# mynameisfiber/baton

Measured on NVIDIA H100. Metric: federated local samples/sec (whole box), ResNet-18 FedAvg, synthetic non-IID 32x32 shards, higher is better.
Workload: dtype bf16

## Files before the change

### baton_b200/csrc/bindings.cpp

```cpp
#include <ATen/cuda/CUDAContext.h>
#include <c10/cuda/CUDAGuard.h>
#include <torch/extension.h>

#include <optional>
#include <vector>

#include "launch.h"

namespace {

inline cudaStream_t cur_stream() { return at::cuda::getCurrentCUDAStream().stream(); }
inline void check(int rc, const char* what) {
  TORCH_CHECK(rc == 0, "baton_b200::", what, " failed with code ", rc,
              rc > 0 ? std::string(" (") + cudaGetErrorString(static_cast<cudaError_t>(rc)) + ")" : std::string());
}
inline const void* cptr(const at::Tensor& t) { return t.data_ptr(); }
inline void* ptr(at::Tensor& t) { return t.data_ptr(); }
template <class T>
inline T* opt_ptr(const std::optional<at::Tensor>& t) {
  return (t.has_value() && t->defined()) ? reinterpret_cast<T*>(t->data_ptr()) : nullptr;
}
#define CHECK_CUDA(x) TORCH_CHECK((x).is_cuda(), #x " must be a CUDA tensor")

inline const float* prox_anchor(const std::optional<at::Tensor>& anchor, int64_t numel, const at::Tensor& hyper) {
// ... 248 lines not shown
  return true;
}
bool conv_smallmap(const at::Tensor& src, const at::Tensor& w, at::Tensor out, int64_t stride, bool dgrad, int64_t mc,
                   int64_t bn, const std::optional<at::Tensor>& col_stats) {
  CHECK_CUDA(src); CHECK_CUDA(w); CHECK_CUDA(out);
  TORCH_CHECK(src.scalar_type() == at::kBFloat16 && w.scalar_type() == at::kBFloat16 && out.scalar_type() == at::kBFloat16 &&
              src.dim() == 4 && src.is_contiguous() && w.is_contiguous() && out.is_contiguous());
  TORCH_CHECK(stride == 1 || stride == 2, "conv_smallmap: stride 1 or 2");
  const int64_t c = src.size(3);
  const int64_t rows = src.size(0) * ((src.size(1) - 1) / stride + 1) * ((src.size(2) - 1) / stride + 1);
  TORCH_CHECK(rows > 0 && out.numel() % rows == 0, "conv_smallmap: out must hold [N*Ho*Wo, Nout] elements");
  const int64_t nout = out.numel() / rows;
  TORCH_CHECK(w.numel() == (dgrad ? c * 9 * nout : nout * 9 * c), "conv_smallmap: w must be [Cout, 9*Cin]");
  TORCH_CHECK(dgrad ? !col_stats.has_value()
                    : (!col_stats.has_value() || (col_stats->scalar_type() == at::kFloat && col_stats->numel() >= 2 * nout)),
              "conv_smallmap: col_stats is a [2 Cout] fp32 buffer of the forward");
  const c10::cuda::CUDAGuard guard(src.device());
  const int rc = b200_conv_smallmap(cptr(src), cptr(w), ptr(out), static_cast<int>(src.size(0)),
                                    static_cast<int>(src.size(1)), static_cast<int>(src.size(2)), static_cast<int>(c),
                                    static_cast<int>(nout), static_cast<int>(stride), dgrad ? 1 : 0, static_cast<int>(mc),
                                    static_cast<int>(bn), opt_ptr<float>(col_stats), cur_stream());
  if (rc == -2) return false;
  check(rc, "conv_smallmap");
  return true;
}
bool conv_igemm_dgrad_s2(const at::Tensor& dy, const at::Tensor& w, at::Tensor dx, int64_t kh, int64_t kw,
                         const std::vector<int64_t>& ntaps, const std::vector<int64_t>& taps, int64_t force_bn) {
  CHECK_CUDA(dy); CHECK_CUDA(w); CHECK_CUDA(dx);
  TORCH_CHECK(dy.scalar_type() == at::kBFloat16 && w.scalar_type() == at::kBFloat16 && dx.scalar_type() == at::kBFloat16 &&
              dy.dim() == 4 && dx.dim() == 4 && dy.is_contiguous() && w.is_contiguous() && dx.is_contiguous());
  TORCH_CHECK(ntaps.size() == 4 && taps.size() == 16, "conv_igemm_dgrad_s2: 4 classes x 4 taps");
  int nt[4], tw[16];
  for (int i = 0; i < 4; ++i) nt[i] = static_cast<int>(ntaps[i]);
  for (int i = 0; i < 16; ++i) tw[i] = static_cast<int>(taps[i]);
  const c10::cuda::CUDAGuard guard(dy.device());
  const int rc = b200_conv_igemm_dgrad_s2(cptr(dy), cptr(w), ptr(dx), static_cast<int>(dx.size(0)),
                                          static_cast<int>(dx.size(1)), static_cast<int>(dx.size(2)),
                                          static_cast<int>(dx.size(3)), static_cast<int>(dy.size(3)), static_cast<int>(kh),
                                          static_cast<int>(kw), static_cast<int>(dy.size(1)), static_cast<int>(dy.size(2)),
                                          nt, tw, static_cast<int>(force_bn), cur_stream());
  if (rc == -2) return false;
  check(rc, "conv_igemm_dgrad_s2");
  return true;
}
bool conv_igemm_wgrad(const at::Tensor& dy, const at::Tensor& x, at::Tensor dw, int64_t cout, int64_t kh, int64_t kw,
                      int64_t stride, int64_t pad, int64_t ho, int64_t wo, int64_t split_k, int64_t force_bn,
// ... 1201 lines not shown

PYBIND11_MODULE(TORCH_EXTENSION_NAME, m) {
  m.doc() = "baton_b200 sm_90a kernels";
  m.attr("MAX_RANKS") = B200_MAX_RANKS;
  m.def("gemm", &gemm);
  m.def("gemm_lora", &gemm_lora);
  m.def("lora_down", &lora_down);
  m.def("lora_grad", &lora_grad);
  m.attr("LORA_MAX_R") = B200_LORA_MAX_R;
  m.attr("LORA_SPLIT_ROWS") = B200_LORA_SPLIT_ROWS;
  m.def("trace_set", &trace_set);
  m.def("attention_fwd", &attention_fwd);
  m.def("attention_bwd", &attention_bwd);
  m.def("bn_bwd_cluster", &bn_bwd_cluster);
  m.def("gn_fwd", &gn_fwd);
  m.def("gn_bwd", &gn_bwd);
  m.def("im2col_tma_probe", &im2col_tma_probe);
  m.def("conv_igemm_fwd", &conv_igemm_fwd);
  m.def("conv_igemm_wgrad", &conv_igemm_wgrad);
  m.def("conv_igemm_dgrad", &conv_igemm_dgrad);
  m.def("conv_igemm_dgrad_s2", &conv_igemm_dgrad_s2);
  m.def("conv_halo", &conv_halo);
  m.def("conv_smallmap", &conv_smallmap);
  m.def("gemm_batched", &gemm_batched);
  m.def("gemm_fp8", &gemm_fp8);
  m.def("quant_mx_rows", &quant_mx_rows);
  m.def("quant_mx_cols", &quant_mx_cols);
  m.def("fused_sgd", &fused_sgd);
  m.def("fused_sgd_segments", &fused_sgd_segments);
  m.def("grad_norm_clip", &grad_norm_clip);
  m.attr("GRAD_NORM_WORK_WORDS") = B200_GRAD_NORM_WORK_WORDS;
  m.def("weighted_sum", &weighted_sum);
  m.def("fold_client", &fold_client);
  m.def("scaffold_corr", &scaffold_corr);
  m.def("scaffold_dc", &scaffold_dc);
  m.def("cast", &cast);
  m.def("gather_rows", &gather_rows);
  m.def("gather_augment", &gather_augment);
  m.def("gather_mix", &gather_mix);
  m.def("colsum", &colsum);
  m.def("add_bf16", &add_bf16);
  m.def("relu_bwd", &relu_bwd);
  m.def("gelu", &gelu);
  m.def("gelu_bwd", &gelu_bwd);
  m.def("pad_rows", &pad_rows);
  m.def("embedding_bwd", &embedding_bwd);
// ... 51 lines not shown
```

### baton_b200/csrc/conv_halo.cu

```cuda
#define B200_TU_TAG 12
#include "ptx.cuh"
#include "epilogue.cuh"
#include "launch.h"
#include "pdl.cuh"

namespace b200 {

constexpr int HALO_BM = 64;
constexpr int HALO_BN = 64;
constexpr int HALO_TAPS = 9;
constexpr int HALO_THREADS = 256;
constexpr int HALO_CONSUMERS = 128;
constexpr int HALO_MAX_SMEM = 227 * 1024;
constexpr int HALO_ZERO_BYTES = 128;

struct HaloParams {
  int M, N;
  int Ho, Wo;
  __nv_bfloat16* D;
  float* col_stats;
  int ncol;
  int mc;
  int halo_bytes;
  int bh, bw;
};

__host__ __device__ constexpr int halo_barriers(int k_tiles) { return (1 + k_tiles + 15) / 16 * 16; }

__host__ __device__ constexpr int halo_slot_bytes(int bn) { return bn * 64 * 2; }

__host__ __device__ constexpr int halo_fixed_bytes(int k_tiles, int bn = HALO_BN, bool img = false) {
  return k_tiles * halo_slot_bytes(bn) + halo_barriers(k_tiles) * 8 + 4 * bn * 4 + (img ? HALO_ZERO_BYTES : 0) + 1024;
}

template <bool DGRAD, int CB, int STRIDE, int BN = HALO_BN, bool IMG = false>
__global__ void __launch_bounds__(HALO_THREADS, 1)
conv_halo_kernel(const __grid_constant__ CUtensorMap tmX, const __grid_constant__ CUtensorMap tmW, const HaloParams p) {
  static_assert(BN == 32 || BN == 64, "conv_halo_kernel: 32 or 64 columns");
  constexpr int KT = HALO_TAPS * CB;
  constexpr int SLOT = halo_slot_bytes(BN);
  constexpr int PITCH = BN + 4;
  constexpr int ORIGIN = IMG ? 0 : -1;
  extern __shared__ __align__(1024) uint8_t smem_raw[];
  uint8_t* smem = reinterpret_cast<uint8_t*>((reinterpret_cast<uintptr_t>(smem_raw) + 1023) & ~uintptr_t(1023));
  uint8_t* halo = smem;
  uint8_t* bslot = smem + CB * p.halo_bytes;
  uint64_t* bar = reinterpret_cast<uint64_t*>(bslot + KT * SLOT);
  float* cstat = reinterpret_cast<float*>(bar + halo_barriers(KT));
  uint8_t* zline = reinterpret_cast<uint8_t*>(cstat + 4 * BN);

  griddep_launch_dependents();
  const int warp = threadIdx.x >> 5;
  const int m0 = blockIdx.y * HALO_BM;
  const int n0 = blockIdx.x * BN;
  const int hw = p.Ho * p.Wo;
  const int hp = p.bh, wp = p.bw;

  if (warp == 0 && elect_one()) {
    tma_prefetch_desc(&tmX);
    tma_prefetch_desc(&tmW);
    for (int i = 0; i < 1 + KT; ++i) mbar_init(&bar[i], 1);
    fence_barrier_init();
  }
  __syncthreads();
  if (p.mc > 1) cluster_sync_all();
  griddep_wait();

  if (warp == 0) {
    if (elect_one()) {
      const int imgs = HALO_BM / hw;
      mbar_expect_tx(&bar[0], CB * imgs * hp * wp * 128);
#pragma unroll
      for (int cb = 0; cb < CB; ++cb)
        tma_load_4d(halo + cb * p.halo_bytes, &tmX, &bar[0], 64 * cb, ORIGIN, ORIGIN, m0 / hw);
      constexpr int SROWS = DGRAD ? 64 : BN;
      constexpr int RB = SLOT / SROWS;
      const int rows = max(SROWS / p.mc, 8);
      const int rank = p.mc > 1 ? static_cast<int>(cluster_ctarank()) : 0;
      const uint16_t mask = static_cast<uint16_t>((1u << p.mc) - 1);
#pragma unroll 1
      for (int kt = 0; kt < KT; ++kt) {
        const int tap = kt / CB, cb = kt - tap * CB;
        mbar_expect_tx(&bar[1 + kt], SLOT);
        if (rank * rows >= SROWS) continue;
        uint8_t* dst = bslot + kt * SLOT + rank * rows * RB;
        const int c0 = DGRAD ? (HALO_TAPS - 1 - tap) * p.ncol + n0 : kt * 64;
        const int c1 = DGRAD ? cb * 64 + rank * rows : n0 + rank * rows;
        if (p.mc > 1)
          tma_load_2d_mc(dst, &tmW, &bar[1 + kt], c0, c1, mask);
        else
          tma_load_2d(dst, &tmW, &bar[1 + kt], c0, c1);
      }
    }
  } else if (warp >= 4) {
    const int ew = warp - 4;
    const int lane = static_cast<int>(lane_id());
    const int m = 16 * ew + (lane & 15);
    const int img = m / hw, rem = m - img * hw;
    const int oi = rem / p.Wo, oj = rem - oi * p.Wo;
    const int y0 = STRIDE * oi - 1 - ORIGIN, x0 = STRIDE * oj - 1 - ORIGIN;
    const int hrow0 = (img * hp + y0) * wp + x0;
    const uint32_t halo_a = smem_u32(halo);
    const int half = lane >> 4;
    auto load_a = [&](uint32_t (&a)[4][4], int kt) {
      const int tap = kt / CB, cb = kt - tap * CB;
      const int r = tap / 3, s = tap - 3 * r;
      const int hrow = hrow0 + r * wp + s;
      uint32_t row_addr = halo_a + static_cast<uint32_t>(cb * p.halo_bytes + hrow * 128);
      if constexpr (IMG) {
        const int y = y0 + r, x = x0 + s;
        if (y < 0 || y >= hp || x < 0 || x >= wp) row_addr = smem_u32(zline);
      }
#pragma unroll
      for (int kk = 0; kk < 4; ++kk) ldmatrix_x4(a[kk], row_addr + ((((2 * kk + half) ^ hrow) & 7) << 4));
    };

    float acc[BN / 2];
#pragma unroll
    for (int j = 0; j < BN / 2; ++j) acc[j] = 0.f;
    uint32_t a[2][4][4];
    if constexpr (IMG) {
      if (threadIdx.x < 128 + HALO_ZERO_BYTES / 16) reinterpret_cast<uint4*>(zline)[threadIdx.x - 128] = make_uint4(0, 0, 0, 0);
      named_bar_sync(1, HALO_CONSUMERS);
    }
    mbar_wait(&bar[0], 0);
    if (threadIdx.x == 128) TRACE_POINT();
    load_a(a[0], 0);
#pragma unroll
    for (int kt = 0; kt < KT; ++kt) {
      mbar_wait(&bar[1 + kt], 0);
      if (threadIdx.x == 128 && (kt == 0 || kt == KT - 1)) TRACE_POINT();
      const uint32_t sb = smem_u32(bslot + kt * SLOT);
      wgmma_fence();
#pragma unroll
      for (int kk = 0; kk < 4; ++kk) {
        uint64_t bd;
        if constexpr (!DGRAD)
          bd = gmma_desc_sw128(sb + kk * 32, 16, 1024);
        else if constexpr (BN == 64)
          bd = gmma_desc_sw128(sb + kk * 2048, 8192, 1024);
        else
          bd = gmma_desc_sw64(sb + kk * 1024, 4096, 512);
        if constexpr (BN == 64)
          wgmma_bf16_n64_rs<DGRAD ? 1 : 0>(acc, a[kt & 1][kk], bd, 1u);
        else
          wgmma_bf16_n32_rs<DGRAD ? 1 : 0>(acc, a[kt & 1][kk], bd, 1u);
      }
      wgmma_commit();
      if (kt + 1 < KT) {
        wgmma_wait<1>();
        load_a(a[(kt + 1) & 1], kt + 1);
      }
    }
    wgmma_wait<0>();
    wgmma_fence_operands(acc);
    if (threadIdx.x == 128) TRACE_POINT();

    named_bar_sync(1, HALO_CONSUMERS);
    float* part = reinterpret_cast<float*>(smem);
    wg_store_acc<BN>(acc, part, PITCH, 0);
    named_bar_sync(1, HALO_CONSUMERS);
    const int q = ew & 1;
    const int c = (ew >> 1) * 32;
    const int lrow = q * 32 + lane;
    const int row = m0 + lrow;
    const int col0 = n0 + c;
    float* sstat = cstat + q * 2 * BN;
    const bool want_stats = p.col_stats != nullptr;
    if (c >= BN) {
    } else if (col0 >= p.N) {
      if (want_stats) { sstat[c + lane] = 0.f; sstat[BN + c + lane] = 0.f; }
    } else {
      uint32_t r[32];
      acc_ld_row32(part + lrow * PITCH + c, r);
      float v[32];
#pragma unroll
      for (int j = 0; j < 32; ++j) v[j] = __uint_as_float(r[j]);
      if (want_stats) stage_col_stats(sstat, BN, c, v);
      if (row < p.M) {
        __nv_bfloat16* d = p.D + static_cast<size_t>(row) * p.N + col0;
        if (col0 + 32 <= p.N && (p.N % 8) == 0) {
#pragma unroll
          for (int j = 0; j < 32; j += 8) {
            uint4 o;
            o.x = pack_bf16x2(v[j], v[j + 1]);
            o.y = pack_bf16x2(v[j + 2], v[j + 3]);
            o.z = pack_bf16x2(v[j + 4], v[j + 5]);
            o.w = pack_bf16x2(v[j + 6], v[j + 7]);
            *reinterpret_cast<uint4*>(d + j) = o;
          }
        } else {
          _Pragma("unroll") for (int j = 0; j < 32; ++j) if (col0 + j < p.N) d[j] = __float2bfloat16_rn(v[j]);
        }
      }
    }
    if (want_stats) {
      named_bar_sync(1, HALO_CONSUMERS);
      for (int i = threadIdx.x - 128; i < 2 * BN; i += HALO_CONSUMERS) {
        const int col = i < BN ? i : i - BN;
        if (n0 + col < p.N)
          atomicAdd(p.col_stats + (i < BN ? 0 : p.N) + n0 + col,
                    cstat[i] + cstat[2 * BN + i]);
      }
    }
  }
}

template <auto KERNEL>
static int launch_halo(const CUtensorMap& tx, const CUtensorMap& tw, const HaloParams& p, dim3 grid, int smem,
                       cudaStream_t stream) {
  static bool configured = false;
  if (!configured) {
    cudaError_t e = cudaFuncSetAttribute(KERNEL, cudaFuncAttributeMaxDynamicSharedMemorySize,
                                         HALO_MAX_SMEM);
    if (e != cudaSuccess) return static_cast<int>(e);
    configured = true;
  }
  cudaLaunchConfig_t cfg = {};
  cfg.gridDim = grid;
// ... 2 lines not shown
  cfg.stream = stream;
  cudaLaunchAttribute attr[2];
  int na = 0;
  if (pdl_enabled()) {
    attr[na].id = cudaLaunchAttributeProgrammaticStreamSerialization;
    attr[na].val.programmaticStreamSerializationAllowed = 1;
    ++na;
  }
  if (p.mc > 1) {
    attr[na].id = cudaLaunchAttributeClusterDimension;
    attr[na].val.clusterDim.x = 1;
    attr[na].val.clusterDim.y = p.mc;
    attr[na].val.clusterDim.z = 1;
    ++na;
  }
  cfg.attrs = attr;
  cfg.numAttrs = na;
  cudaError_t le = cudaLaunchKernelEx(&cfg, KERNEL, tx, tw, p);
  if (le != cudaSuccess) return static_cast<int>(le);
  return static_cast<int>(cudaGetLastError());
}

static int conv_tiled_setup(const void* src, const void* w, void* out, int N, int H, int W, int C, int Nout, int stride,
                            int dgrad, int mc, int bn, bool img, float* col_stats, CUtensorMap* tx, CUtensorMap* tw,
                            HaloParams* p, dim3* grid, int* smem);

}

extern "C" int b200_encode_map2_bf16(void* map, const void* base, long long rows, long long cols, long long ld,
                                     int box_cols, int box_rows);
extern "C" int b200_encode_map2_sw64_bf16(void* map, const void* base, long long rows, long long cols, long long ld,
                                          int box_cols, int box_rows);
extern "C" int b200_encode_map4_box_bf16(void* map, const void* base, const long long* dims,
                                         const long long* stride_bytes, const int* box);

namespace b200 {

static int conv_tiled_setup(const void* src, const void* w, void* out, int N, int H, int W, int C, int Nout, int stride,
                            int dgrad, int mc, int bn, bool img, float* col_stats, CUtensorMap* tx, CUtensorMap* tw,
                            HaloParams* p, dim3* grid, int* smem) {
  const int Ho = (H - 1) / stride + 1, Wo = (W - 1) / stride + 1;
  const long long M = static_cast<long long>(N) * Ho * Wo;
  if (M <= 0 || Nout <= 0) return 1;
  const int hw = Ho * Wo;
  const long long m_tiles = (M + HALO_BM - 1) / HALO_BM;
  const int bh = img ? H : stride * (Ho - 1) + 3, bw = img ? W : stride * (Wo - 1) + 3;
  if (H <= 0 || W <= 0 || HALO_BM % hw != 0 || bh > 256 || bw > 256 || M > (1ll << 30) || Nout % 8 != 0 ||
      ((dgrad || img) && Nout % bn != 0) || (mc != 1 && mc != 2 && mc != 4 && mc != 8) || m_tiles % mc != 0 ||
      (reinterpret_cast<uintptr_t>(src) & 15) || (reinterpret_cast<uintptr_t>(w) & 15) ||
      (reinterpret_cast<uintptr_t>(out) & 15))
    return -2;
  const int imgs = HALO_BM / hw;
  const int cb = C / 64;
  const int box_bytes = (imgs * bh * bw * 128 + 1023) / 1024 * 1024;
  *smem = cb * box_bytes + halo_fixed_bytes(HALO_TAPS * cb, bn, img);
  if (*smem > HALO_MAX_SMEM) return -2;
  const long long dims[4] = {C, W, H, N};
  const long long strides[3] = {static_cast<long long>(C) * 2, static_cast<long long>(W) * C * 2,
                                static_cast<long long>(H) * W * C * 2};
  const int box[4] = {64, bw, bh, imgs};
  int rc = b200_encode_map4_box_bf16(tx, src, dims, strides, box);
  if (rc) return rc;
  const long long wrows = dgrad ? C : Nout, wcols = dgrad ? 9ll * Nout : 9ll * C;
  const int srows = dgrad ? 64 : bn;
  const int rows = srows / mc > 8 ? srows / mc : 8;
  rc = dgrad && bn == 32 ? b200_encode_map2_sw64_bf16(tw, w, wrows, wcols, wcols, bn, rows)
                         : b200_encode_map2_bf16(tw, w, wrows, wcols, wcols, dgrad ? bn : 64, rows);
  if (rc) return rc;
  p->M = static_cast<int>(M); p->N = Nout; p->Ho = Ho; p->Wo = Wo; p->D = reinterpret_cast<__nv_bfloat16*>(out);
  p->col_stats = col_stats; p->ncol = Nout; p->mc = mc; p->halo_bytes = box_bytes; p->bh = bh; p->bw = bw;
  *grid = dim3((Nout + bn - 1) / bn, static_cast<unsigned>(m_tiles), 1);
  return 0;
}

}

extern "C" int b200_conv_halo(const void* src, const void* w, void* out, int N, int H, int W, int C, int Nout,
                              int stride, int dgrad, int mc, float* col_stats, cudaStream_t stream) {
  using namespace b200;
  const bool s1c64 = stride == 1 && C == 64, s1c128 = stride == 1 && C == 128, s2c64 = stride == 2 && C == 64 && !dgrad;
  if (!s1c64 && !s1c128 && !s2c64) return -2;
  CUtensorMap tx, tw;
  HaloParams p;
  dim3 grid;
  int smem = 0;
  const int rc = conv_tiled_setup(src, w, out, N, H, W, C, Nout, stride, dgrad, mc, HALO_BN, false, col_stats, &tx, &tw,
                                  &p, &grid, &smem);
  if (rc) return rc == 1 ? 0 : rc;
  if (s2c64) return launch_halo<conv_halo_kernel<false, 1, 2>>(tx, tw, p, grid, smem, stream);
  if (s1c64)
    return dgrad ? launch_halo<conv_halo_kernel<true, 1, 1>>(tx, tw, p, grid, smem, stream)
                 : launch_halo<conv_halo_kernel<false, 1, 1>>(tx, tw, p, grid, smem, stream);
  return dgrad ? launch_halo<conv_halo_kernel<true, 2, 1>>(tx, tw, p, grid, smem, stream)
               : launch_halo<conv_halo_kernel<false, 2, 1>>(tx, tw, p, grid, smem, stream);
}

extern "C" int b200_conv_smallmap(const void* src, const void* w, void* out, int N, int H, int W, int C, int Nout,
                                  int stride, int dgrad, int mc, int bn, float* col_stats, cudaStream_t stream) {
  using namespace b200;
  const bool s1c256 = stride == 1 && C == 256 && bn == 32;
  const bool s2c128 = stride == 2 && C == 128 && !dgrad && (bn == 32 || bn == 64);
  if (!s1c256 && !s2c128) return -2;
  CUtensorMap tx, tw;
  HaloParams p;
  dim3 grid;
  int smem = 0;
  const int rc = conv_tiled_setup(src, w, out, N, H, W, C, Nout, stride, dgrad, mc, bn, true, col_stats, &tx, &tw, &p,
                                  &grid, &smem);
  if (rc) return rc == 1 ? 0 : rc;
  if (s2c128)
    return bn == 32 ? launch_halo<conv_halo_kernel<false, 2, 2, 32, true>>(tx, tw, p, grid, smem, stream)
                    : launch_halo<conv_halo_kernel<false, 2, 2, 64, true>>(tx, tw, p, grid, smem, stream);
  return dgrad ? launch_halo<conv_halo_kernel<true, 4, 1, 32, true>>(tx, tw, p, grid, smem, stream)
               : launch_halo<conv_halo_kernel<false, 4, 1, 32, true>>(tx, tw, p, grid, smem, stream);
}

B200_TRACE_REGISTER(conv_halo)
```

### baton_b200/csrc/launch.h

```cpp
#pragma once
#include <cuda_runtime.h>
#include <stdint.h>

#define B200_MAX_RANKS 16

extern "C" {

struct B200SgdEpilogue {
  float* theta;
  void* theta_bf16;
  float* mom;
  const float* hyper;
  int nesterov;
  const float* anchor;
  const float* corr;
  float* v;
};
#define B200_SGD_EPILOGUE_DECLINED (-6)

struct B200AffineEpilogue {
  const float* scale;
  const float* shift;
  const void* residual;
  long long ldr;
// ... 33 lines not shown
int b200_attention_fwd(const void* qkv, void* out, void* probs, int B, int S, int H, int dh, float scale,
                       cudaStream_t stream);
int b200_attention_bwd(const void* qkv, const void* dout, const void* probs, void* dqkv, int B, int S, int H, int dh,
                       float scale, cudaStream_t stream);
struct B200Dropout;
int b200_attention_drop_fwd(const void* qkv, void* out, void* probs, int B, int S, int H, int dh, float scale,
                            const B200Dropout* drop, cudaStream_t stream);
int b200_attention_drop_bwd(const void* qkv, const void* dout, const void* probs, void* dqkv, int B, int S, int H, int dh,
                            float scale, const B200Dropout* drop, cudaStream_t stream);
int b200_conv_igemm_fwd(const void* x, const void* w, void* y, int N, int H, int W, int Cin, int Cout, int KH, int KW,
                        int stride, int pad, int Ho, int Wo, int cluster_k, int force_bn, float* col_stats,
                        const B200AffineEpilogue* affine, cudaStream_t stream);
int b200_conv_igemm_dgrad(const void* dy, const void* w, void* dx, int N, int H, int W, int Cin, int Cout, int KH, int KW,
                          int pad, int Ho, int Wo, int cluster_k, int force_bn, cudaStream_t stream);
int b200_conv_igemm_dgrad_s2(const void* dy, const void* w, void* dx, int N, int H, int W, int Cin, int Cout, int KH,
                             int KW, int Ho, int Wo, const int* ntaps, const int* taps, int force_bn, cudaStream_t stream);
int b200_conv_igemm_wgrad(const void* dy, const void* x, float* dw, int N, int H, int W, int Cin, int Cout, int KH, int KW,
                          int stride, int pad, int Ho, int Wo, int split_k, int force_bn, const B200SgdEpilogue* sgd,
                          cudaStream_t stream);
int b200_conv_halo(const void* src, const void* w, void* out, int N, int H, int W, int C, int Nout, int stride,
                   int dgrad, int mc, float* col_stats, cudaStream_t stream);
int b200_conv_smallmap(const void* src, const void* w, void* out, int N, int H, int W, int C, int Nout, int stride,
                       int dgrad, int mc, int bn, float* col_stats, cudaStream_t stream);
int b200_im2col_tma_probe(const void* x, void* col, int N, int H, int W, int C, int KH, int KW, int stride, int pad,
                          int Ho, int Wo, cudaStream_t stream);
int b200_gemm_fp8(const void* a, const void* b, void* d, const float* bias, const void* sfa, const void* sfb, int M, int N,
                  int K, long long lda, long long ldb, long long ldd, int out_fp32, int act, int split_k, int accumulate,
                  float alpha, cudaStream_t stream);
int b200_quant_mx_rows(const void* x, void* q, void* sf, long long R, int C, long long ld_in, int Cp, cudaStream_t stream);
int b200_quant_mx_cols(const void* x, void* q, void* sf, long long R, int C, long long ld_in, long long Rp,
                       cudaStream_t stream);
int b200_gemm_simt(const void* a, const void* b, void* d, const float* bias, int M, int N, int K, long long lda,
                   long long ldb, long long ldd, int a_mn, int b_mn, int out_fp32, int act, int accumulate,
                   float alpha, cudaStream_t stream);

int b200_fused_sgd(float* w, float* g, float* mom, void* w_bf16, long long n, const float* hyper, int zero_grad,
                   int nesterov, const unsigned long long* wire_slot, const float* pack_global,
                   const float* pack_scale, long long n_pack, int wire_fp32, const float* prox_anchor,
                   const float* corr, float* adam_v, int clip, cudaStream_t stream);
int b200_fused_sgd_segments(float* w, float* g, float* mom, void* w_bf16, const long long* segments, int n_seg,
                            const float* hyper, int nesterov, const float* prox_anchor, const float* corr,
                            float* adam_v, int clip, cudaStream_t stream);
#define B200_GRAD_NORM_BLOCKS 528
#define B200_GRAD_NORM_WORK_WORDS (B200_GRAD_NORM_BLOCKS + 2)
int b200_grad_norm_clip(const float* g, long long n, const float* max_norm, void* work, float* norm_out,
                        float* coef_out, cudaStream_t stream);
// ... 232 lines not shown
```

### baton_b200/ops/functional.py

```python
from __future__ import annotations

import collections
import functools
from typing import List, Optional, Sequence, Tuple

import torch

from ._ext import load

BF16 = torch.bfloat16
NUM_SMS = 132


def _pitch(t: torch.Tensor) -> int:
    assert t.dim() == 2 and (t.stride(1) == 1 or t.shape[1] == 1), "GEMM operand must have unit inner stride"
    return t.stride(0) if t.shape[0] > 1 else max(t.stride(0), t.shape[1])


def _tma_ok(t: torch.Tensor) -> bool:
    return t.dtype == BF16 and _pitch(t) % 8 == 0 and t.data_ptr() % 16 == 0


def pick_bn(M: int, N: int) -> int:
    m_tiles = (M + 127) // 128
# ... 428 lines not shown


HALO_BM = 64
_HALO_MAX_SMEM = 227 * 1024
_HALO_FORMS = ((1, 64), (1, 128), (2, 64))


def halo_smem_bytes(h: int, w: int, c: int = 64, stride: int = 1) -> int:
    ho, wo = conv_out_size(h, 3, stride, 1), conv_out_size(w, 3, stride, 1)
    box = (HALO_BM // (ho * wo)) * (stride * (ho - 1) + 3) * (stride * (wo - 1) + 3) * 128
    k_tiles = 9 * (c // 64)
    return c // 64 * round_up(box, 1024) + k_tiles * 8192 + round_up(1 + k_tiles, 16) * 8 + 4 * 64 * 4 + 1024


def halo_eligible(kh: int, kw: int, stride: int, pad: int, c: int, h: int, w: int,
                  affine: Optional[dict] = None, dgrad: bool = False) -> bool:
    if kh != 3 or kw != 3 or pad != 1 or (stride, c) not in _HALO_FORMS or (dgrad and stride != 1):
        return False
    hw = conv_out_size(h, 3, stride, 1) * conv_out_size(w, 3, stride, 1)
    return (hw <= HALO_BM and HALO_BM % hw == 0 and affine is None and
            halo_smem_bytes(h, w, c, stride) <= _HALO_MAX_SMEM)


def halo_cluster(m_rows: int) -> int:
    tiles = (m_rows + HALO_BM - 1) // HALO_BM
    return 4 if tiles % 4 == 0 else 2 if tiles % 2 == 0 else 1


_SMALLMAP_FORMS = ((1, 256), (2, 128))
SMALLMAP_BN = 32


def smallmap_smem_bytes(h: int, w: int, c: int = 256, stride: int = 1, bn: int = SMALLMAP_BN) -> int:
    ho, wo = conv_out_size(h, 3, stride, 1), conv_out_size(w, 3, stride, 1)
    box = (HALO_BM // (ho * wo)) * h * w * 128
    k_tiles = 9 * (c // 64)
    return (c // 64 * round_up(box, 1024) + k_tiles * bn * 128 + round_up(1 + k_tiles, 16) * 8 + 4 * bn * 4 + 128
            + 1024)


def smallmap_eligible(kh: int, kw: int, stride: int, pad: int, c: int, h: int, w: int,
                      affine: Optional[dict] = None, dgrad: bool = False) -> bool:
    if kh != 3 or kw != 3 or pad != 1 or (stride, c) not in _SMALLMAP_FORMS or (dgrad and stride != 1):
        return False
    hw = conv_out_size(h, 3, stride, 1) * conv_out_size(w, 3, stride, 1)
    return (hw <= HALO_BM and HALO_BM % hw == 0 and affine is None and
            smallmap_smem_bytes(h, w, c, stride) <= _HALO_MAX_SMEM)


def _conv_path(path: Optional[str], eligible: bool, smallmap: bool = False) -> str:
    if path is None:
        return "halo" if eligible else "smallmap" if smallmap else "im2col"
    if path not in ("halo", "smallmap", "im2col"):
        raise ValueError("path must be None, 'halo', 'smallmap' or 'im2col', not {!r}".format(path))
    if path == "halo" and not eligible:
        raise ValueError("the halo kernel does not take this convolution (see halo_eligible)")
    if path == "smallmap" and not smallmap:
        raise ValueError("the image-tile kernel does not take this convolution (see smallmap_eligible)")
    return path


def conv_igemm_fwd(x: torch.Tensor, w2d: torch.Tensor, kh: int, kw: int, stride: int, pad: int,
                   col_stats: Optional[torch.Tensor] = None, affine: Optional[dict] = None,
                   cluster_k: Optional[int] = None, force_bn: int = 0,
                   out: Optional[torch.Tensor] = None, path: Optional[str] = None,
                   mc: Optional[int] = None, bn: int = SMALLMAP_BN) -> Optional[torch.Tensor]:
    n, h, w, c = x.shape
    cout = w2d.shape[0]
    if c % 64 or w2d.shape[1] != kh * kw * c or not x.is_contiguous() or not w2d.is_contiguous():
        return None
    ho, wo = conv_out_size(h, kh, stride, pad), conv_out_size(w, kw, stride, pad)
    M, K = n * ho * wo, kh * kw * c
    halo = halo_eligible(kh, kw, stride, pad, c, h, w, affine) and cout % 8 == 0
    small = smallmap_eligible(kh, kw, stride, pad, c, h, w, affine) and cout % bn == 0
    kind = _conv_path(path, halo, small)
    if kind == "halo":
        y = out if out is not None else torch.empty((M, cout), dtype=BF16, device=x.device)
        if not load().conv_halo(x, w2d, y, stride, False, mc or halo_cluster(M), col_stats):
            raise RuntimeError("conv_halo declined a convolution halo_eligible admits")
        return y
    if kind == "smallmap":
# ... 25 lines not shown
                dp = (a + pad - r) // 2
                for s in range(kw):
                    if (b + pad - s) % 2:
                        continue
                    dq = (b + pad - s) // 2
                    if dp < 0 or dq < 0:
                        return None
                    if dp < ho and dq < wo:
                        taps.append((r * kw + s, dp, dq))
            if len(taps) > S2_MAX_TAPS:
                return None
            classes.append(taps)
    return classes


def conv_igemm_dgrad(dy: torch.Tensor, w2d: torch.Tensor, in_shape, kh: int, kw: int, pad: int, stride: int = 1,
                     out: Optional[torch.Tensor] = None, path: Optional[str] = None,
                     mc: Optional[int] = None, cluster_k: Optional[int] = None) -> Optional[torch.Tensor]:
    n, h, w, c = in_shape
    cout = dy.shape[-1]
    if c % 64 or cout % 64 or w2d.shape[1] != kh * kw * c or not dy.is_contiguous() or not w2d.is_contiguous():
        return None
    kind = _conv_path(path, halo_eligible(kh, kw, stride, pad, cout, h, w, dgrad=True),
                      smallmap_eligible(kh, kw, stride, pad, cout, h, w, dgrad=True) and c % SMALLMAP_BN == 0)
    if kind == "halo":
        dx = out if out is not None else torch.empty((n, h, w, c), dtype=BF16, device=dy.device)
        if not load().conv_halo(dy, w2d, dx, 1, True, mc or halo_cluster(n * h * w), None):
            raise RuntimeError("conv_halo declined a convolution halo_eligible admits")
        return dx
    if kind == "smallmap":
        dx = out if out is not None else torch.empty((n, h, w, c), dtype=BF16, device=dy.device)
        if not load().conv_smallmap(dy, w2d, dx, 1, True, mc or halo_cluster(n * h * w), SMALLMAP_BN, None):
            raise RuntimeError("conv_smallmap declined a convolution smallmap_eligible admits")
        return dx
    if stride == 1:
        M, K = n * h * w, kh * kw * cout
        bn = pick_bn(M, c)
        dx = out if out is not None else torch.empty((n, h, w, c), dtype=BF16, device=dy.device)
        if cluster_k is None:
            cluster_k = pick_cluster_k(M, c, K, bn)
        ok = load().conv_igemm_dgrad(dy, w2d, dx, kh, kw, pad, cluster_k, bn)
        return dx if ok else None
    if stride != 2:
        return None
    ho, wo = dy.shape[1], dy.shape[2]
    classes = conv_s2_dgrad_taps(kh, kw, pad, ho, wo)
    if classes is None:
        return None
    bn = pick_bn(4 * n * ho * wo, c)
    words = [[t | dp << 16 | dq << 24 for t, dp, dq in taps] + [0] * (S2_MAX_TAPS - len(taps)) for taps in classes]
    dx = out if out is not None else torch.empty((n, h, w, c), dtype=BF16, device=dy.device)
    ok = load().conv_igemm_dgrad_s2(dy, w2d, dx, kh, kw, [len(t) for t in classes], [x for ws in words for x in ws], bn)
    return dx if ok else None


def conv_igemm_wgrad_(dy2d: torch.Tensor, x: torch.Tensor, dw2d: torch.Tensor, kh: int, kw: int, stride: int,
                      pad: int, sgd: Optional[dict] = None) -> bool:
    n, h, w, c = x.shape
    cout = dy2d.shape[1]
    if c % 64 or not x.is_contiguous() or not dy2d.is_contiguous() or not dw2d.is_contiguous():
        return False
    ho, wo = conv_out_size(h, kh, stride, pad), conv_out_size(w, kw, stride, pad)
    M, K = n * ho * wo, kh * kw * c
    bn = pick_bn(cout, K)
    split_k = pick_split_k(cout, K, M, bn)
    if sgd is not None and split_k != 1:
        return False
    sg = sgd or {}
    return bool(load().conv_igemm_wgrad(dy2d, x, dw2d, cout, kh, kw, stride, pad, ho, wo, split_k, bn,
                                        sg.get("theta"), sg.get("theta_bf16"), sg.get("momentum"), sg.get("hyper"),
                                        bool(sg.get("nesterov", False)), sg.get("anchor"), sg.get("corr"),
                                        sg.get("adam_v")))


def col2im(col: torch.Tensor, shape: Tuple[int, int, int, int], kh: int, kw: int, stride: int, pad: int,
           ho: int, wo: int) -> torch.Tensor:
# ... 192 lines not shown
```

Measured before the change: 230,200.

## Add image-mode halo kernel for stride-2 3x3 conv dgrad on small maps

Adds a stride-2 dgrad path to the halo conv kernel. Each CTA takes one output parity class, loads whole dy images into shared memory via TMA, and runs only that class's valid taps. Each CTA covers two 64-row passes and scatters rows to the interleaved dx positions. For the ResNet-18 small-map downsample layers this replaces the general im2col-style s2 igemm path, aiming for less global traffic and fewer wasted taps. It needs extra shared memory for a partial-sum buffer, and eligibility is limited to Cout of 128, 256 or 512 with small spatial maps.

```diff
diff --git a/baton_b200/csrc/bindings.cpp b/baton_b200/csrc/bindings.cpp
--- a/baton_b200/csrc/bindings.cpp
+++ b/baton_b200/csrc/bindings.cpp
@@ -294,6 +294,26 @@
                                     static_cast<int>(bn), opt_ptr<float>(col_stats), cur_stream());
   if (rc == -2) return false;
   check(rc, "conv_smallmap");
+  return true;
+}
+bool conv_s2_image(const at::Tensor& dy, const at::Tensor& w, at::Tensor dx, int64_t mc, const std::vector<int64_t>& ntaps,
+                   const std::vector<int64_t>& taps) {
+  CHECK_CUDA(dy); CHECK_CUDA(w); CHECK_CUDA(dx);
+  TORCH_CHECK(dy.scalar_type() == at::kBFloat16 && w.scalar_type() == at::kBFloat16 && dx.scalar_type() == at::kBFloat16 &&
+              dy.dim() == 4 && dx.dim() == 4 && dy.is_contiguous() && w.is_contiguous() && dx.is_contiguous());
+  TORCH_CHECK(dy.size(0) == dx.size(0) && w.numel() == dy.size(3) * 9 * dx.size(3),
+              "conv_s2_image: dy [N, Ho, Wo, Cout], w [Cout, 9*Cin], dx [N, H, W, Cin]");
+  TORCH_CHECK(ntaps.size() == 4 && taps.size() == 16, "conv_s2_image: 4 classes x 4 taps");
+  int nt[4], tw[16];
+  for (int i = 0; i < 4; ++i) nt[i] = static_cast<int>(ntaps[i]);
+  for (int i = 0; i < 16; ++i) tw[i] = static_cast<int>(taps[i]);
+  const c10::cuda::CUDAGuard guard(dy.device());
+  const int rc = b200_conv_s2_image(cptr(dy), cptr(w), ptr(dx), static_cast<int>(dx.size(0)), static_cast<int>(dx.size(1)),
+                                    static_cast<int>(dx.size(2)), static_cast<int>(dx.size(3)),
+                                    static_cast<int>(dy.size(3)), static_cast<int>(dy.size(1)),
+                                    static_cast<int>(dy.size(2)), static_cast<int>(mc), nt, tw, cur_stream());
+  if (rc == -2) return false;
+  check(rc, "conv_s2_image");
   return true;
 }
 bool conv_igemm_dgrad_s2(const at::Tensor& dy, const at::Tensor& w, at::Tensor dx, int64_t kh, int64_t kw,
@@ -1541,6 +1561,7 @@
   m.def("conv_igemm_dgrad_s2", &conv_igemm_dgrad_s2);
   m.def("conv_halo", &conv_halo);
   m.def("conv_smallmap", &conv_smallmap);
+  m.def("conv_s2_image", &conv_s2_image);
   m.def("gemm_batched", &gemm_batched);
   m.def("gemm_fp8", &gemm_fp8);
   m.def("quant_mx_rows", &quant_mx_rows);
diff --git a/baton_b200/csrc/conv_halo.cu b/baton_b200/csrc/conv_halo.cu
--- a/baton_b200/csrc/conv_halo.cu
+++ b/baton_b200/csrc/conv_halo.cu
@@ -13,6 +13,9 @@
 constexpr int HALO_CONSUMERS = 128;
 constexpr int HALO_MAX_SMEM = 227 * 1024;
 constexpr int HALO_ZERO_BYTES = 128;
+
+constexpr int HALO_S2_TAPS = 4;
+constexpr int HALO_S2_PASSES = 2;
 
 struct HaloParams {
   int M, N;
@@ -23,6 +26,10 @@
   int mc;
   int halo_bytes;
   int bh, bw;
+  int slots;
+  int dh, dw;
+  int s2_ntaps[4];
+  int s2_tap[4][HALO_S2_TAPS];
 };
 
 __host__ __device__ constexpr int halo_barriers(int k_tiles) { return (1 + k_tiles + 15) / 16 * 16; }
@@ -37,21 +44,42 @@
 __global__ void __launch_bounds__(HALO_THREADS, 1)
 conv_halo_kernel(const __grid_constant__ CUtensorMap tmX, const __grid_constant__ CUtensorMap tmW, const HaloParams p) {
   static_assert(BN == 32 || BN == 64, "conv_halo_kernel: 32 or 64 columns");
-  constexpr int KT = HALO_TAPS * CB;
+  constexpr bool S2D = DGRAD && STRIDE == 2;
+  static_assert(!S2D || IMG, "conv_halo_kernel: the stride-2 dgrad runs in image mode");
+  constexpr int KT_MAX = S2D ? HALO_S2_TAPS * CB : HALO_TAPS * CB;
   constexpr int SLOT = halo_slot_bytes(BN);
   constexpr int PITCH = BN + 4;
   constexpr int ORIGIN = IMG ? 0 : -1;
+  constexpr int PASSES = S2D ? HALO_S2_PASSES : 1;
+  constexpr int TILE_M = PASSES * HALO_BM;
+  const int nslot = S2D ? p.slots : KT_MAX;
   extern __shared__ __align__(1024) uint8_t smem_raw[];
   uint8_t* smem = reinterpret_cast<uint8_t*>((reinterpret_cast<uintptr_t>(smem_raw) + 1023) & ~uintptr_t(1023));
   uint8_t* halo = smem;
   uint8_t* bslot = smem + CB * p.halo_bytes;
-  uint64_t* bar = reinterpret_cast<uint64_t*>(bslot + KT * SLOT);
-  float* cstat = reinterpret_cast<float*>(bar + halo_barriers(KT));
+  uint64_t* bar = reinterpret_cast<uint64_t*>(bslot + nslot * SLOT);
+  float* cstat = reinterpret_cast<float*>(bar + halo_barriers(nslot));
   uint8_t* zline = reinterpret_cast<uint8_t*>(cstat + 4 * BN);
+  float* part = reinterpret_cast<float*>(PASSES > 1 ? zline + HALO_ZERO_BYTES : smem);
 
   griddep_launch_dependents();
   const int warp = threadIdx.x >> 5;
-  const int m0 = blockIdx.y * HALO_BM;
+  int cls = 0, m0 = blockIdx.y * TILE_M;
+  if constexpr (S2D) {
+    const int tiles_m = (p.M + TILE_M - 1) / TILE_M;
+    cls = static_cast<int>(blockIdx.y) / tiles_m;
+    m0 = (static_cast<int>(blockIdx.y) - cls * tiles_m) * TILE_M;
+  }
+  int kt_n = KT_MAX;
+  int s2w[HALO_S2_TAPS] = {};
+  if constexpr (S2D) {
+#pragma unroll
+    for (int c = 0; c < 4; ++c) {
+      kt_n = c == cls ? p.s2_ntaps[c] * CB : kt_n;
+#pragma unroll
+      for (int t = 0; t < HALO_S2_TAPS; ++t) s2w[t] = c == cls ? p.s2_tap[c][t] : s2w[t];
+    }
+  }
   const int n0 = blockIdx.x * BN;
   const int hw = p.Ho * p.Wo;
   const int hp = p.bh, wp = p.bw;
@@ -59,7 +87,7 @@
   if (warp == 0 && elect_one()) {
     tma_prefetch_desc(&tmX);
     tma_prefetch_desc(&tmW);
-    for (int i = 0; i < 1 + KT; ++i) mbar_init(&bar[i], 1);
+    for (int i = 0; i < 1 + nslot; ++i) mbar_init(&bar[i], 1);
     fence_barrier_init();
   }
   __syncthreads();
@@ -68,7 +96,7 @@
 
   if (warp == 0) {
     if (elect_one()) {
-      const int imgs = HALO_BM / hw;
+      const int imgs = TILE_M / hw;
       mbar_expect_tx(&bar[0], CB * imgs * hp * wp * 128);
 #pragma unroll
       for (int cb = 0; cb < CB; ++cb)
@@ -79,12 +107,17 @@
       const int rank = p.mc > 1 ? static_cast<int>(cluster_ctarank()) : 0;
       const uint16_t mask = static_cast<uint16_t>((1u << p.mc) - 1);
 #pragma unroll 1
-      for (int kt = 0; kt < KT; ++kt) {
+      for (int kt = 0; kt < kt_n; ++kt) {
         const int tap = kt / CB, cb = kt - tap * CB;
         mbar_expect_tx(&bar[1 + kt], SLOT);
         if (rank * rows >= SROWS) continue;
         uint8_t* dst = bslot + kt * SLOT + rank * rows * RB;
-        const int c0 = DGRAD ? (HALO_TAPS - 1 - tap) * p.ncol + n0 : kt * 64;
+        int ftap = HALO_TAPS - 1 - tap;
+        if constexpr (S2D) {
+#pragma unroll
+          for (int t = 0; t < HALO_S2_TAPS; ++t) ftap = t == tap ? (s2w[t] & 0xffff) : ftap;
+        }
+        const int c0 = DGRAD ? ftap * p.ncol + n0 : kt * 64;
         const int c1 = DGRAD ? cb * 64 + rank * rows : n0 + rank * rows;
         if (p.mc > 1)
           tma_load_2d_mc(dst, &tmW, &bar[1 + kt], c0, c1, mask);
@@ -95,106 +128,118 @@
   } else if (warp >= 4) {
     const int ew = warp - 4;
     const int lane = static_cast<int>(lane_id());
-    const int m = 16 * ew + (lane & 15);
-    const int img = m / hw, rem = m - img * hw;
-    const int oi = rem / p.Wo, oj = rem - oi * p.Wo;
-    const int y0 = STRIDE * oi - 1 - ORIGIN, x0 = STRIDE * oj - 1 - ORIGIN;
-    const int hrow0 = (img * hp + y0) * wp + x0;
     const uint32_t halo_a = smem_u32(halo);
     const int half = lane >> 4;
-    auto load_a = [&](uint32_t (&a)[4][4], int kt) {
-      const int tap = kt / CB, cb = kt - tap * CB;
-      const int r = tap / 3, s = tap - 3 * r;
-      const int hrow = hrow0 + r * wp + s;
-      uint32_t row_addr = halo_a + static_cast<uint32_t>(cb * p.halo_bytes + hrow * 128);
-      if constexpr (IMG) {
-        const int y = y0 + r, x = x0 + s;
-        if (y < 0 || y >= hp || x < 0 || x >= wp) row_addr = smem_u32(zline);
-      }
-#pragma unroll
-      for (int kk = 0; kk < 4; ++kk) ldmatrix_x4(a[kk], row_addr + ((((2 * kk + half) ^ hrow) & 7) << 4));
-    };
-
-    float acc[BN / 2];
-#pragma unroll
-    for (int j = 0; j < BN / 2; ++j) acc[j] = 0.f;
-    uint32_t a[2][4][4];
     if constexpr (IMG) {
       if (threadIdx.x < 128 + HALO_ZERO_BYTES / 16) reinterpret_cast<uint4*>(zline)[threadIdx.x - 128] = make_uint4(0, 0, 0, 0);
       named_bar_sync(1, HALO_CONSUMERS);
     }
     mbar_wait(&bar[0], 0);
     if (threadIdx.x == 128) TRACE_POINT();
-    load_a(a[0], 0);
-#pragma unroll
-    for (int kt = 0; kt < KT; ++kt) {
-      mbar_wait(&bar[1 + kt], 0);
-      if (threadIdx.x == 128 && (kt == 0 || kt == KT - 1)) TRACE_POINT();
-      const uint32_t sb = smem_u32(bslot + kt * SLOT);
-      wgmma_fence();
-#pragma unroll
-      for (int kk = 0; kk < 4; ++kk) {
-        uint64_t bd;
-        if constexpr (!DGRAD)
-          bd = gmma_desc_sw128(sb + kk * 32, 16, 1024);
-        else if constexpr (BN == 64)
-          bd = gmma_desc_sw128(sb + kk * 2048, 8192, 1024);
-        else
-          bd = gmma_desc_sw64(sb + kk * 1024, 4096, 512);
-        if constexpr (BN == 64)
-          wgmma_bf16_n64_rs<DGRAD ? 1 : 0>(acc, a[kt & 1][kk], bd, 1u);
-        else
-          wgmma_bf16_n32_rs<DGRAD ? 1 : 0>(acc, a[kt & 1][kk], bd, 1u);
-      }
-      wgmma_commit();
-      if (kt + 1 < KT) {
-        wgmma_wait<1>();
-        load_a(a[(kt + 1) & 1], kt + 1);
-      }
-    }
-    wgmma_wait<0>();
-    wgmma_fence_operands(acc);
-    if (threadIdx.x == 128) TRACE_POINT();
-
-    named_bar_sync(1, HALO_CONSUMERS);
-    float* part = reinterpret_cast<float*>(smem);
-    wg_store_acc<BN>(acc, part, PITCH, 0);
-    named_bar_sync(1, HALO_CONSUMERS);
-    const int q = ew & 1;
-    const int c = (ew >> 1) * 32;
-    const int lrow = q * 32 + lane;
-    const int row = m0 + lrow;
-    const int col0 = n0 + c;
-    float* sstat = cstat + q * 2 * BN;
-    const bool want_stats = p.col_stats != nullptr;
-    if (c >= BN) {
-    } else if (col0 >= p.N) {
-      if (want_stats) { sstat[c + lane] = 0.f; sstat[BN + c + lane] = 0.f; }
-    } else {
-      uint32_t r[32];
-      acc_ld_row32(part + lrow * PITCH + c, r);
-      float v[32];
-#pragma unroll
-      for (int j = 0; j < 32; ++j) v[j] = __uint_as_float(r[j]);
-      if (want_stats) stage_col_stats(sstat, BN, c, v);
-      if (row < p.M) {
-        __nv_bfloat16* d = p.D + static_cast<size_t>(row) * p.N + col0;
-        if (col0 + 32 <= p.N && (p.N % 8) == 0) {
-#pragma unroll
-          for (int j = 0; j < 32; j += 8) {
-            uint4 o;
-            o.x = pack_bf16x2(v[j], v[j + 1]);
-            o.y = pack_bf16x2(v[j + 2], v[j + 3]);
-            o.z = pack_bf16x2(v[j + 4], v[j + 5]);
-            o.w = pack_bf16x2(v[j + 6], v[j + 7]);
-            *reinterpret_cast<uint4*>(d + j) = o;
-          }
-        } else {
-          _Pragma("unroll") for (int j = 0; j < 32; ++j) if (col0 + j < p.N) d[j] = __float2bfloat16_rn(v[j]);
+#pragma unroll 1
+    for (int pass = 0; pass < PASSES; ++pass) {
+      const int mp = pass * HALO_BM;
+      const int m = mp + 16 * ew + (lane & 15);
+      const int img = m / hw, rem = m - img * hw;
+      const int oi = rem / p.Wo, oj = rem - oi * p.Wo;
+      const int y0 = S2D ? oi : STRIDE * oi - 1 - ORIGIN, x0 = S2D ? oj : STRIDE * oj - 1 - ORIGIN;
+      const int hrow0 = (img * hp + y0) * wp + x0;
+      auto load_a = [&](uint32_t (&a)[4][4], int kt) {
+        const int tap = kt / CB, cb = kt - tap * CB;
+        const int r = S2D ? (s2w[tap] >> 16) & 0xff : tap / 3;
+        const int s = S2D ? (s2w[tap] >> 24) & 0xff : tap - 3 * (tap / 3);
+        const int hrow = hrow0 + r * wp + s;
+        uint32_t row_addr = halo_a + static_cast<uint32_t>(cb * p.halo_bytes + hrow * 128);
+        if constexpr (IMG) {
+          const int y = y0 + r, x = x0 + s;
+          if (y < 0 || y >= hp || x < 0 || x >= wp) row_addr = smem_u32(zline);
+        }
+#pragma unroll
+        for (int kk = 0; kk < 4; ++kk) ldmatrix_x4(a[kk], row_addr + ((((2 * kk + half) ^ hrow) & 7) << 4));
+      };
+
+      float acc[BN / 2];
+#pragma unroll
+      for (int j = 0; j < BN / 2; ++j) acc[j] = 0.f;
+      uint32_t a[2][4][4];
+      load_a(a[0], 0);
+#pragma unroll
+      for (int kt = 0; kt < KT_MAX; ++kt) {
+        if (kt >= kt_n) break;
+        mbar_wait(&bar[1 + kt], 0);
+        if (threadIdx.x == 128 && (kt == 0 || kt == kt_n - 1)) TRACE_POINT();
+        const uint32_t sb = smem_u32(bslot + kt * SLOT);
+        wgmma_fence();
+#pragma unroll
+        for (int kk = 0; kk < 4; ++kk) {
+          uint64_t bd;
+          if constexpr (!DGRAD)
+            bd = gmma_desc_sw128(sb + kk * 32, 16, 1024);
+          else if constexpr (BN == 64)
+            bd = gmma_desc_sw128(sb + kk * 2048, 8192, 1024);
+          else
+            bd = gmma_desc_sw64(sb + kk * 1024, 4096, 512);
+          if constexpr (BN == 64)
+            wgmma_bf16_n64_rs<DGRAD ? 1 : 0>(acc, a[kt & 1][kk], bd, 1u);
+          else
+            wgmma_bf16_n32_rs<DGRAD ? 1 : 0>(acc, a[kt & 1][kk], bd, 1u);
+        }
+        wgmma_commit();
+        if (kt + 1 < kt_n) {
+          wgmma_wait<1>();
+          load_a(a[(kt + 1) & 1], kt + 1);
         }
       }
-    }
-    if (want_stats) {
+      wgmma_wait<0>();
+      wgmma_fence_operands(acc);
+      if (threadIdx.x == 128) TRACE_POINT();
+
+      named_bar_sync(1, HALO_CONSUMERS);
+      wg_store_acc<BN>(acc, part, PITCH, 0);
+      named_bar_sync(1, HALO_CONSUMERS);
+      const int q = ew & 1;
+      const int c = (ew >> 1) * 32;
+      const int lrow = q * 32 + lane;
+      const int row = m0 + mp + lrow;
+      int orow = row;
+      if constexpr (S2D) {
+        const int n = row / hw, rr = row - n * hw;
+        const int i = rr / p.Wo, j = rr - i * p.Wo;
+        const int h = 2 * i + (cls >> 1), w = 2 * j + (cls & 1);
+        orow = row < p.M && h < p.dh && w < p.dw ? (n * p.dh + h) * p.dw + w : -1;
+      }
+      const int col0 = n0 + c;
+      float* sstat = cstat + q * 2 * BN;
+      const bool want_stats = p.col_stats != nullptr;
+      if (c >= BN) {
+      } else if (col0 >= p.N) {
+        if (want_stats) { sstat[c + lane] = 0.f; sstat[BN + c + lane] = 0.f; }
+      } else {
+        uint32_t r[32];
+        acc_ld_row32(part + lrow * PITCH + c, r);
+        float v[32];
+#pragma unroll
+        for (int j = 0; j < 32; ++j) v[j] = __uint_as_float(r[j]);
+        if (want_stats) stage_col_stats(sstat, BN, c, v);
+        if (S2D ? orow >= 0 : row < p.M) {
+          __nv_bfloat16* d = p.D + static_cast<size_t>(orow) * p.N + col0;
+          if (col0 + 32 <= p.N && (p.N % 8) == 0) {
+#pragma unroll
+            for (int j = 0; j < 32; j += 8) {
+              uint4 o;
+              o.x = pack_bf16x2(v[j], v[j + 1]);
+              o.y = pack_bf16x2(v[j + 2], v[j + 3]);
+              o.z = pack_bf16x2(v[j + 4], v[j + 5]);
+              o.w = pack_bf16x2(v[j + 6], v[j + 7]);
+              *reinterpret_cast<uint4*>(d + j) = o;
+            }
+          } else {
+            _Pragma("unroll") for (int j = 0; j < 32; ++j) if (col0 + j < p.N) d[j] = __float2bfloat16_rn(v[j]);
+          }
+        }
+      }
+    }
+    if (p.col_stats != nullptr) {
       named_bar_sync(1, HALO_CONSUMERS);
       for (int i = threadIdx.x - 128; i < 2 * BN; i += HALO_CONSUMERS) {
         const int col = i < BN ? i : i - BN;
@@ -243,8 +288,8 @@
 }
 
 static int conv_tiled_setup(const void* src, const void* w, void* out, int N, int H, int W, int C, int Nout, int stride,
-                            int dgrad, int mc, int bn, bool img, float* col_stats, CUtensorMap* tx, CUtensorMap* tw,
-                            HaloParams* p, dim3* grid, int* smem);
+                            int dgrad, int mc, int bn, bool img, int taps, int bm, float* col_stats,
+                            CUtensorMap* tx, CUtensorMap* tw, HaloParams* p, dim3* grid, int* smem);
 
 }
 
@@ -258,23 +303,23 @@
 namespace b200 {
 
 static int conv_tiled_setup(const void* src, const void* w, void* out, int N, int H, int W, int C, int Nout, int stride,
-                            int dgrad, int mc, int bn, bool img, float* col_stats, CUtensorMap* tx, CUtensorMap* tw,
-                            HaloParams* p, dim3* grid, int* smem) {
+                            int dgrad, int mc, int bn, bool img, int taps, int bm, float* col_stats,
+                            CUtensorMap* tx, CUtensorMap* tw, HaloParams* p, dim3* grid, int* smem) {
   const int Ho = (H - 1) / stride + 1, Wo = (W - 1) / stride + 1;
   const long long M = static_cast<long long>(N) * Ho * Wo;
   if (M <= 0 || Nout <= 0) return 1;
   const int hw = Ho * Wo;
-  const long long m_tiles = (M + HALO_BM - 1) / HALO_BM;
+  const long long m_tiles = (M + bm - 1) / bm;
   const int bh = img ? H : stride * (Ho - 1) + 3, bw = img ? W : stride * (Wo - 1) + 3;
-  if (H <= 0 || W <= 0 || HALO_BM % hw != 0 || bh > 256 || bw > 256 || M > (1ll << 30) || Nout % 8 != 0 ||
+  if (H <= 0 || W <= 0 || bm % hw != 0 || bh > 256 || bw > 256 || M > (1ll << 30) || Nout % 8 != 0 ||
       ((dgrad || img) && Nout % bn != 0) || (mc != 1 && mc != 2 && mc != 4 && mc != 8) || m_tiles % mc != 0 ||
       (reinterpret_cast<uintptr_t>(src) & 15) || (reinterpret_cast<uintptr_t>(w) & 15) ||
       (reinterpret_cast<uintptr_t>(out) & 15))
     return -2;
-  const int imgs = HALO_BM / hw;
+  const int imgs = bm / hw;
   const int cb = C / 64;
   const int box_bytes = (imgs * bh * bw * 128 + 1023) / 1024 * 1024;
-  *smem = cb * box_bytes + halo_fixed_bytes(HALO_TAPS * cb, bn, img);
+  *smem = cb * box_bytes + halo_fixed_bytes(taps * cb, bn, img);
   if (*smem > HALO_MAX_SMEM) return -2;
   const long long dims[4] = {C, W, H, N};
   const long long strides[3] = {static_cast<long long>(C) * 2, static_cast<long long>(W) * C * 2,
@@ -290,6 +335,7 @@
   if (rc) return rc;
   p->M = static_cast<int>(M); p->N = Nout; p->Ho = Ho; p->Wo = Wo; p->D = reinterpret_cast<__nv_bfloat16*>(out);
   p->col_stats = col_stats; p->ncol = Nout; p->mc = mc; p->halo_bytes = box_bytes; p->bh = bh; p->bw = bw;
+  p->slots = taps * cb; p->dh = H; p->dw = W;
   *grid = dim3((Nout + bn - 1) / bn, static_cast<unsigned>(m_tiles), 1);
   return 0;
 }
@@ -305,8 +351,8 @@
   HaloParams p;
   dim3 grid;
   int smem = 0;
-  const int rc = conv_tiled_setup(src, w, out, N, H, W, C, Nout, stride, dgrad, mc, HALO_BN, false, col_stats, &tx, &tw,
-                                  &p, &grid, &smem);
+  const int rc = conv_tiled_setup(src, w, out, N, H, W, C, Nout, stride, dgrad, mc, HALO_BN, false, HALO_TAPS, HALO_BM,
+                                  col_stats, &tx, &tw, &p, &grid, &smem);
   if (rc) return rc == 1 ? 0 : rc;
   if (s2c64) return launch_halo<conv_halo_kernel<false, 1, 2>>(tx, tw, p, grid, smem, stream);
   if (s1c64)
@@ -326,8 +372,8 @@
   HaloParams p;
   dim3 grid;
   int smem = 0;
-  const int rc = conv_tiled_setup(src, w, out, N, H, W, C, Nout, stride, dgrad, mc, bn, true, col_stats, &tx, &tw, &p,
-                                  &grid, &smem);
+  const int rc = conv_tiled_setup(src, w, out, N, H, W, C, Nout, stride, dgrad, mc, bn, true, HALO_TAPS, HALO_BM,
+                                  col_stats, &tx, &tw, &p, &grid, &smem);
   if (rc) return rc == 1 ? 0 : rc;
   if (s2c128)
     return bn == 32 ? launch_halo<conv_halo_kernel<false, 2, 2, 32, true>>(tx, tw, p, grid, smem, stream)
@@ -336,4 +382,40 @@
                : launch_halo<conv_halo_kernel<false, 4, 1, 32, true>>(tx, tw, p, grid, smem, stream);
 }
 
+extern "C" int b200_conv_s2_image(const void* dy, const void* w, void* dx, int N, int H, int W, int Cin, int Cout,
+                                  int Ho, int Wo, int mc, const int* ntaps, const int* taps, cudaStream_t stream) {
+  using namespace b200;
+  if (Cout != 128 && Cout != 256 && Cout != 512) return -2;
+  if ((H + 1) / 2 != Ho || (W + 1) / 2 != Wo) return -2;
+  int max_taps = 0;
+  for (int c = 0; c < 4; ++c) {
+    if (ntaps[c] < 0 || ntaps[c] > HALO_S2_TAPS) return -2;
+    for (int t = 0; t < ntaps[c]; ++t) {
+      const int tw = taps[c * HALO_S2_TAPS + t];
+      if (tw < 0 || (tw & 0xffff) >= HALO_TAPS || ((tw >> 16) & 0xff) > 1 || ((tw >> 24) & 0xff) > 1) return -2;
+    }
+    max_taps = ntaps[c] > max_taps ? ntaps[c] : max_taps;
+  }
+  if (max_taps == 0) return -2;
+  CUtensorMap tx, tw;
+  HaloParams p;
+  dim3 grid;
+  int smem = 0;
+  const int rc = conv_tiled_setup(dy, w, dx, N, Ho, Wo, Cout, Cin, 1, 1, mc, HALO_BN, true, max_taps,
+                                  HALO_S2_PASSES * HALO_BM, nullptr, &tx, &tw, &p, &grid, &smem);
+  if (rc) return rc == 1 ? 0 : rc;
+  smem += HALO_BM * (HALO_BN + 4) * 4;
+  if (smem > HALO_MAX_SMEM) return -2;
+  if (4ll * grid.y > 65535) return -2;
+  grid.y *= 4;
+  p.dh = H; p.dw = W;
+  for (int c = 0; c < 4; ++c) {
+    p.s2_ntaps[c] = ntaps[c];
+    for (int t = 0; t < HALO_S2_TAPS; ++t) p.s2_tap[c][t] = t < ntaps[c] ? taps[c * HALO_S2_TAPS + t] : 0;
+  }
+  if (Cout == 128) return launch_halo<conv_halo_kernel<true, 2, 2, 64, true>>(tx, tw, p, grid, smem, stream);
+  if (Cout == 256) return launch_halo<conv_halo_kernel<true, 4, 2, 64, true>>(tx, tw, p, grid, smem, stream);
+  return launch_halo<conv_halo_kernel<true, 8, 2, 64, true>>(tx, tw, p, grid, smem, stream);
+}
+
 B200_TRACE_REGISTER(conv_halo)
diff --git a/baton_b200/csrc/launch.h b/baton_b200/csrc/launch.h
--- a/baton_b200/csrc/launch.h
+++ b/baton_b200/csrc/launch.h
@@ -79,6 +79,8 @@
                    int dgrad, int mc, float* col_stats, cudaStream_t stream);
 int b200_conv_smallmap(const void* src, const void* w, void* out, int N, int H, int W, int C, int Nout, int stride,
                        int dgrad, int mc, int bn, float* col_stats, cudaStream_t stream);
+int b200_conv_s2_image(const void* dy, const void* w, void* dx, int N, int H, int W, int Cin, int Cout, int Ho, int Wo,
+                       int mc, const int* ntaps, const int* taps, cudaStream_t stream);
 int b200_im2col_tma_probe(const void* x, void* col, int N, int H, int W, int C, int KH, int KW, int stride, int pad,
                           int Ho, int Wo, cudaStream_t stream);
 int b200_gemm_fp8(const void* a, const void* b, void* d, const float* bias, const void* sfa, const void* sfb, int M, int N,
diff --git a/baton_b200/ops/functional.py b/baton_b200/ops/functional.py
--- a/baton_b200/ops/functional.py
+++ b/baton_b200/ops/functional.py
@@ -474,8 +474,8 @@
             halo_smem_bytes(h, w, c, stride) <= _HALO_MAX_SMEM)
 
 
-def halo_cluster(m_rows: int) -> int:
-    tiles = (m_rows + HALO_BM - 1) // HALO_BM
+def halo_cluster(m_rows: int, bm: int = HALO_BM) -> int:
+    tiles = (m_rows + bm - 1) // bm
     return 4 if tiles % 4 == 0 else 2 if tiles % 2 == 0 else 1
 
 
@@ -500,15 +500,37 @@
             smallmap_smem_bytes(h, w, c, stride) <= _HALO_MAX_SMEM)
 
 
-def _conv_path(path: Optional[str], eligible: bool, smallmap: bool = False) -> str:
+_S2_IMAGE_FORMS = (128, 256, 512)
+S2_IMAGE_BM = 2 * HALO_BM
+
+
+def s2_image_smem_bytes(h: int, w: int, cout: int) -> int:
+    ho, wo = conv_out_size(h, 3, 2, 1), conv_out_size(w, 3, 2, 1)
+    box = (S2_IMAGE_BM // (ho * wo)) * ho * wo * 128
+    k_tiles = max(len(t) for t in conv_s2_dgrad_taps(3, 3, 1, ho, wo)) * (cout // 64)
+    return (cout // 64 * round_up(box, 1024) + k_tiles * 8192 + round_up(1 + k_tiles, 16) * 8 + 4 * 64 * 4 + 128
+            + HALO_BM * 68 * 4 + 1024)
+
+
+def s2_image_eligible(kh: int, kw: int, stride: int, pad: int, c: int, h: int, w: int,
+                      affine: Optional[dict] = None, dgrad: bool = False) -> bool:
+    if not dgrad or kh != 3 or kw != 3 or stride != 2 or pad != 1 or c not in _S2_IMAGE_FORMS or affine is not None:
+        return False
+    hw = conv_out_size(h, 3, 2, 1) * conv_out_size(w, 3, 2, 1)
+    return hw <= HALO_BM and HALO_BM % hw == 0 and s2_image_smem_bytes(h, w, c) <= _HALO_MAX_SMEM
+
+
+def _conv_path(path: Optional[str], eligible: bool, smallmap: bool = False, s2image: bool = False) -> str:
     if path is None:
-        return "halo" if eligible else "smallmap" if smallmap else "im2col"
-    if path not in ("halo", "smallmap", "im2col"):
-        raise ValueError("path must be None, 'halo', 'smallmap' or 'im2col', not {!r}".format(path))
+        return "halo" if eligible else "smallmap" if smallmap else "s2image" if s2image else "im2col"
+    if path not in ("halo", "smallmap", "s2image", "im2col"):
+        raise ValueError("path must be None, 'halo', 'smallmap', 's2image' or 'im2col', not {!r}".format(path))
     if path == "halo" and not eligible:
         raise ValueError("the halo kernel does not take this convolution (see halo_eligible)")
     if path == "smallmap" and not smallmap:
         raise ValueError("the image-tile kernel does not take this convolution (see smallmap_eligible)")
+    if path == "s2image" and not s2image:
+        raise ValueError("the stride-2 image-mode dgrad does not take this convolution (see s2_image_eligible)")
     return path
 
 
@@ -580,7 +602,15 @@
     if c % 64 or cout % 64 or w2d.shape[1] != kh * kw * c or not dy.is_contiguous() or not w2d.is_contiguous():
         return None
     kind = _conv_path(path, halo_eligible(kh, kw, stride, pad, cout, h, w, dgrad=True),
-                      smallmap_eligible(kh, kw, stride, pad, cout, h, w, dgrad=True) and c % SMALLMAP_BN == 0)
+                      smallmap_eligible(kh, kw, stride, pad, cout, h, w, dgrad=True) and c % SMALLMAP_BN == 0,
+                      s2_image_eligible(kh, kw, stride, pad, cout, h, w, dgrad=True))
+    if kind == "s2image":
+        ntaps, words = _s2_tap_words(conv_s2_dgrad_taps(kh, kw, pad, dy.shape[1], dy.shape[2]))
+        dx = out if out is not None else torch.empty((n, h, w, c), dtype=BF16, device=dy.device)
+        rows = dy.shape[0] * dy.shape[1] * dy.shape[2]
+        if not load().conv_s2_image(dy, w2d, dx, mc or halo_cluster(rows, S2_IMAGE_BM), ntaps, words):
+            raise RuntimeError("conv_s2_image declined a convolution s2_image_eligible admits")
+        return dx
     if kind == "halo":
         dx = out if out is not None else torch.empty((n, h, w, c), dtype=BF16, device=dy.device)
         if not load().conv_halo(dy, w2d, dx, 1, True, mc or halo_cluster(n * h * w), None):
@@ -606,10 +636,15 @@
     if classes is None:
         return None
     bn = pick_bn(4 * n * ho * wo, c)
+    ntaps, words = _s2_tap_words(classes)
+    dx = out if out is not None else torch.empty((n, h, w, c), dtype=BF16, device=dy.device)
+    ok = load().conv_igemm_dgrad_s2(dy, w2d, dx, kh, kw, ntaps, words, bn)
+    return dx if ok else None
+
+
+def _s2_tap_words(classes: List[List[Tuple[int, int, int]]]) -> Tuple[List[int], List[int]]:
     words = [[t | dp << 16 | dq << 24 for t, dp, dq in taps] + [0] * (S2_MAX_TAPS - len(taps)) for taps in classes]
-    dx = out if out is not None else torch.empty((n, h, w, c), dtype=BF16, device=dy.device)
-    ok = load().conv_igemm_dgrad_s2(dy, w2d, dx, kh, kw, [len(t) for t in classes], [x for ws in words for x in ws], bn)
-    return dx if ok else None
+    return [len(t) for t in classes], [x for ws in words for x in ws]
 
 
 def conv_igemm_wgrad_(dy2d: torch.Tensor, x: torch.Tensor, dw2d: torch.Tensor, kh: int, kw: int, stride: int,
```

Result: faster. 232,800 (median of 6 runs) (+1.1%).
